# sj-shoff/ImageProcessor

Measured on AMD Instinct MI355X. Metric: images/sec (resize+thumb+watermark) on 1080p batch at 1/2/4/8 MI355X, higher is better.
Workload: dtype f32+f64

## Files before the change

### imageprocessor_amd/csrc/ipx_ks.h

```cpp
#pragma once

#include <vector>

#include "ipx_internal.h"

namespace ipx {

struct KsAxis {
    int dw = 0, sw = 0;
    int ntap = 0;
    std::vector<int32_t> lo, cnt;
    std::vector<double> w;
    std::vector<double> itw, itwffff;
    std::vector<double> ones;
};
bool ks_build_axis(int dw, int sw, KsAxis *out);

struct KsAxisDev {
    const int32_t *lo, *cnt;
    const double *w, *itw, *itwffff, *ones;
    int ntap;
};
size_t ks_axis_bytes(const KsAxis &a);
void ks_axis_pack(const KsAxis &a, uint8_t *h, const uint8_t *d, KsAxisDev *out);
// ... 18 lines not shown
    KsAxisDev ax, ay;
    int op;
    const int *opaque_flag;
    int kind;
    const uint8_t *src; int sstride; size_t src_fs;
    const uint8_t *cb, *cr; int cstride, ratio; size_t c_fs;
    int nframes;
};
hipError_t launch_ks_generic(const KsGenArgs &a, hipStream_t s);

}

namespace ipx {

struct KsStrip { int c0, c1, t0, tw; };
struct KsSeg { int ys, r0, r1; };
template <int NACC> struct KsRowT { double w[NACC], itw[NACC], ones[NACC]; int32_t emit[NACC]; float wf[NACC]; };
static_assert(sizeof(KsRowT<2>) == 64 && sizeof(KsRowT<4>) == 128, "row entries are copied dword-wise");

struct KsFusedOut {
    uint8_t *out; size_t frame_stride; int ostride, obytes;
    int dw, dh, sr_x0, sr_y0;
    int kind;
    int mode, aone;
    int pk;
    int ntap;
    int waves, cpl;
    int wcols;
    const double *wx;
    const float *wxf;
    int split, ntapf;
    float feps;
    const double *itwf;
    const int32_t *xlo;
    const int32_t *colb;
    const void *rows;
    const int32_t *rowoff;
};
struct KsFusedArgs {
    const uint8_t *src; size_t src_fs; int sstride, sw, sh;
    int src_kind;
    int taps_le_alpha;
    const uint8_t *cb, *cr; int cstride, ratio; size_t c_fs;
    uint8_t *wm; size_t wm_fs; int wm_stride;
    int nframes, nstrips, nseg, nthreads, pitch, dbuf;
    const KsStrip *strips; const KsSeg *segs;
    int nout; KsFusedOut o[2];
    int lds_w[2], lds_rows, lds_open;
    int open_per_wave;
    uint8_t wave_role[16];
    unsigned long long *stamps;
    int *redo;
    uint2 *fix; int *fix_count; int fix_cap[2], fix_stride;
};
struct KsFix { uint2 *list = nullptr; int *count = nullptr; int cap[2] = {0, 0}; KsAxisDev ax[2], ay[2]; };
struct KsFusedGeom { int nseg = 0; const KsSeg *segs = nullptr; const void *rows[2] = {nullptr, nullptr}; const int32_t *rowoff[2] = {nullptr, nullptr}; };
struct KsFusedPlan {
    bool ok = false;
    int nacc = 2, rows = 4, pitch = 0, nstrips = 0, nthreads = 0, nstg = 0, dbuf = 0;
    int lds_w[2] = {0, 0}, lds_rows = 0, lds_open = 0, lds_bytes = 0;
    struct Lds { int dbuf = 0, lds_w[2] = {0, 0}, lds_rows = 0, lds_open = 0, open_per_wave = 0, lds_bytes = 0; } fast;
    const KsStrip *strips = nullptr;
    struct Out { int ntap = 0, waves = 0, cpl = 0, wcols = 0; const double *wx = nullptr, *itwf = nullptr; const int32_t *xlo = nullptr, *colb = nullptr;
                 const float *wxf = nullptr; float feps = 0; int split = 1, ntapf = 0; } o[2];
    KsFusedGeom whole, split;
};
constexpr int kKsSplitRows = 96;
constexpr int kKsRows = 4;
constexpr int kKsMaxStage = 3;
constexpr int kKsMaxWaves = 12;
constexpr int kKsMaxThreads = 64 * kKsMaxWaves;
constexpr int kKsMaxCpl = 2;
constexpr int kKsSplitTaps = 16;
constexpr int kKsOpenPerWave = 128;
struct KsFusedIn { int dw, dh, sr_x0, sr_y0; const KsAxis *hx, *hy; int top_taps = 0; };
bool ks_fused_plan(int sw, int sh, const KsFusedIn *sc0, const KsFusedIn *sc1, int px_bytes, std::vector<uint8_t> *blob, KsFusedPlan *out);
void ks_fused_rebase(KsFusedPlan *p, const uint8_t *dev_blob);
hipError_t launch_ks_fused(const KsFusedPlan &p, KsFusedArgs &a, const KsFix *fix, int cus, hipStream_t s, bool *matched);
hipError_t launch_ks_fix(const KsGenArgs &g, const uint2 *list, size_t list_stride, const int *count, int count_stride, int cap, hipStream_t s);

}
```

### imageprocessor_amd/csrc/ipx_ks_fused.hip

```cpp
#include <algorithm>
#include <cstdio>
#include <cstdlib>
#include <type_traits>

#include "ipx_ks.h"

#pragma clang fp contract(off)

#include "ipx_device.h"

namespace ipx {
namespace {

#ifndef IPX_DIAG
#define IPX_DIAG 0
#endif
#if IPX_DIAG
#define KS_DIAG_ARGS , tsum, tlast
#define KS_STAMP(i) do { const unsigned long long t_ = __builtin_amdgcn_s_memtime(); tsum[i] += t_ - tlast; tlast = t_; } while (0)
#else
#define KS_DIAG_ARGS
#define KS_STAMP(i) do { } while (0)
#endif
constexpr int kOOB = 0x7fffffff;

__device__ __forceinline__ void ks_barrier() { asm volatile("s_waitcnt lgkmcnt(0)\n\ts_barrier" ::: "memory"); }
typedef uint32_t u32x4 __attribute__((ext_vector_type(4)));

__device__ __forceinline__ uint32_t ks_ftou8(double f)
{
    int i = (int)(0xffff * f + 0.5);
    i = min(max(i, 0), 0xffff);
    return (uint32_t)i >> 8;
}

enum { KS_RGBA = 0, KS_NRGBA = 1, KS_YCC = 2, KS_GRAY = 3, KS_TAP64 = 4 };
template <int SRC> struct KsPx { static constexpr int bytes = SRC == KS_RGBA ? 4 : SRC == KS_GRAY ? 2 : 8; };
enum { KS_TAP_PLAIN = 0,
       KS_TAP_CLAMP = 1,
       KS_TAP_TOP = 2,
       KS_TAP_MINTOP = 3 };

struct KsStageRegs { uint32_t v[4]; };

__device__ __forceinline__ void ks_ycc16(uint32_t yb, int rt, int gt, int bt, uint32_t &r, uint32_t &g, uint32_t &b)
{
    const int yy1 = (int)(yb * 0x10101u);
    r = (uint32_t)min(max((yy1 + rt) >> 8, 0), 0xffff);
    g = (uint32_t)min(max((yy1 + gt) >> 8, 0), 0xffff);
    b = (uint32_t)min(max((yy1 + bt) >> 8, 0), 0xffff);
}

template <int SRC>
// ... 391 lines not shown
                    }
                }
            }
        }
    }
}

template <int SRC, int NCH, int NACC, int B, bool OPQ, bool RAG, bool FAST>
__global__ __launch_bounds__(kKsMaxThreads) void ks_fused_kernel(KsFusedArgs a)
{
    typedef std::conditional_t<FAST, float, double> Sum;
    constexpr int CPLM = NACC == 2 ? kKsMaxCpl : 1;
    extern __shared__ __align__(16) uint8_t lds[];
    constexpr int PXB = KsPx<SRC>::bytes;
    constexpr int CHB = 4 * PXB;
    const int tid = (int)threadIdx.x, lane = tid & 63, wv = tid >> 6;
    int item = (int)blockIdx.x;
    if (!OPQ && !FAST && a.redo && !a.redo[item]) return;
    const int seg = item % a.nseg;
    item /= a.nseg;
    const int strip = item % a.nstrips, frame = item / a.nstrips;
    const KsStrip st = a.strips[strip];
    const KsSeg sg = a.segs[seg];
    const int pitch = a.pitch, CH = pitch / CHB;
    typedef KsRowT<NACC> Row;
    constexpr int RW = (int)(sizeof(Row) / 4);
    constexpr int SPX = SRC == KS_RGBA || SRC == KS_NRGBA ? 4 : SRC == KS_TAP64 ? 8 : 1;
    const int hs = SRC == KS_YCC && (a.ratio == IPX_YCBCR_422 || a.ratio == IPX_YCBCR_420), vs = SRC == KS_YCC && (a.ratio == IPX_YCBCR_420 || a.ratio == IPX_YCBCR_440);

    const uint8_t *sframe = a.src + (size_t)frame * a.src_fs;
    const __amdgpu_buffer_rsrc_t srs = __builtin_amdgcn_make_buffer_rsrc((void *)sframe, 0, (a.sh - 1) * a.sstride + a.sw * SPX, 0x00020000);
    const int chh = vs ? (a.sh + 1) / 2 : a.sh, cww = hs ? (a.sw + 1) / 2 : a.sw;
    const __amdgpu_buffer_rsrc_t cbrs = __builtin_amdgcn_make_buffer_rsrc((void *)(SRC == KS_YCC ? a.cb + (size_t)frame * a.c_fs : nullptr), 0,
                                                                         SRC == KS_YCC ? (chh - 1) * a.cstride + cww : 0, 0x00020000);
    const __amdgpu_buffer_rsrc_t crrs = __builtin_amdgcn_make_buffer_rsrc((void *)(SRC == KS_YCC ? a.cr + (size_t)frame * a.c_fs : nullptr), 0,
                                                                         SRC == KS_YCC ? (chh - 1) * a.cstride + cww : 0, 0x00020000);
    const __amdgpu_buffer_rsrc_t wrs = __builtin_amdgcn_make_buffer_rsrc((void *)(a.wm ? a.wm + (size_t)frame * a.wm_fs : nullptr), 0,
                                                                        a.wm ? (a.sh - 1) * a.wm_stride + a.sw * 4 : 0, 0x00020000);

    int s_lds[kKsMaxStage], s_src[kKsMaxStage], s_wm[kKsMaxStage], s_row[kKsMaxStage], s_cx[kKsMaxStage], s_np[kKsMaxStage];
    constexpr bool ragged = RAG && (SRC == KS_RGBA || SRC == KS_NRGBA);
#pragma unroll
    for (int i = 0; i < kKsMaxStage; i++) {
        const int q = tid + i * a.nthreads;
        const int row = q / CH, ch = q - row * CH, x = st.t0 + ch * 4;
        const bool in = q < B * CH && x < a.sw;
        s_row[i] = in ? row : -1;
        s_lds[i] = row * pitch + ch * CHB;
        s_src[i] = in ? row * a.sstride + x * SPX : kOOB;
        s_cx[i] = in ? (hs ? x >> 1 : x) : kOOB;
        s_np[i] = !ragged ? 4 : in ? min(4, a.sw - x) : 0;
        s_wm[i] = in && x >= st.c0 && x < st.c1 ? row * a.wm_stride + x * 4 : kOOB;
    }
    const int rk = tid / (B * RW), ri = tid - rk * (B * RW);
    const bool rstage = rk < a.nout;
    const uint32_t *rsrc = rstage ? (const uint32_t *)a.o[rk].rows + (size_t)a.o[rk].rowoff[seg] * RW + ri : nullptr;

    int role = -1, wk = 0;
    {
        const int rb = a.wave_role[wv & 15];
        if (rb != 0xff) { role = rb >> 4; wk = rb & 15; }
    }
    role = __builtin_amdgcn_readfirstlane(role);
    wk = __builtin_amdgcn_readfirstlane(wk);
    KsCol<NCH, NACC, Sum> col[CPLM];
    __amdgpu_buffer_rsrc_t ors = __builtin_amdgcn_make_buffer_rsrc((void *)nullptr, 0, 0, 0x00020000);
    int ntap = 0, wstride = 0, ostride = 0, cpl = 0, mode = KS_TAP_PLAIN;
    float feps = 0.f;
    bool split2 = false;
    bool aone = false;
    const uint8_t *rows_lds = lds + a.lds_rows;
    const int dbuf = a.dbuf;
    const int tile_bytes = B * pitch, rows_bytes = 2 * B * (int)sizeof(Row);
    if (role >= 0) {
        const KsFusedOut &o = a.o[role];
        ors = __builtin_amdgcn_make_buffer_rsrc((void *)(o.out + (size_t)frame * o.frame_stride), 0, o.obytes, 0x00020000);
        split2 = FAST && o.split == 2;
        ntap = FAST ? (split2 ? o.ntapf >> 1 : o.ntapf) : o.ntap;
        wstride = o.wcols * (FAST ? 4 : 8); ostride = o.ostride; cpl = o.cpl; feps = o.feps;
        mode = o.mode; aone = o.aone != 0;
        rows_lds += role * B * (int)sizeof(Row);
        const int cb = o.colb[strip], ce = o.colb[strip + 1];
        {
            const int n = (FAST ? o.ntapf : o.ntap) * o.wcols;
            if (FAST) {
                const float *wsrc = o.wxf + (size_t)strip * o.ntapf * o.wcols;
                float *wdst = (float *)(lds + a.lds_w[role]);
                for (int i = wk * 64 + lane; i < n; i += o.waves * 64) wdst[i] = wsrc[i];
            } else {
                const double *wsrc = o.wx + (size_t)strip * o.ntap * o.wcols;
                double *wdst = (double *)(lds + a.lds_w[role]);
                for (int i = wk * 64 + lane; i < n; i += o.waves * 64) wdst[i] = wsrc[i];
            }
        }
#pragma unroll
        for (int j = 0; j < CPLM; j++) {
            const int slot = wk * 64 + lane + j * 64 * o.waves;
            const int part = split2 ? slot & 1 : 0, cslot = split2 ? slot >> 1 : slot, dx = cb + cslot;
            const bool has = j < o.cpl && dx < ce;
            col[j].clear();
            col[j].itwf = has ? o.itwf[dx] : 0.0;
            col[j].xb = has ? (o.sr_x0 + o.xlo[dx] - st.t0 + part * ntap) * PXB : 0;
            col[j].wofs = a.lds_w[role] + (has ? cslot : 0) * (FAST ? 4 : 8) + part * ntap * wstride;
            col[j].ooff = has && part == 0 ? dx * 4 : kOOB;
        }
    }

    const int ngroups = (sg.r1 - sg.ys + B - 1) / B;
    KsStageRegs stage[kKsMaxStage];
    uint32_t stage2[SRC == KS_TAP64 ? kKsMaxStage : 1][4];
    uint32_t rstg = 0;
    auto issue = [&](int g) {
        const int y0 = sg.ys + g * B;
#pragma unroll
        for (int i = 0; i < kKsMaxStage; i++) {
            const bool ok = s_row[i] >= 0 && y0 + s_row[i] < sg.r1;
            const int off = ok ? s_src[i] : kOOB;
            if (SRC == KS_RGBA || SRC == KS_NRGBA || SRC == KS_TAP64) {
                u32x4 v = __builtin_amdgcn_raw_buffer_load_b128(srs, ragged && s_np[i] < 4 ? kOOB : off, y0 * a.sstride, 0);
                if (ragged) {
                    const int np = ok ? s_np[i] : 4;
                    v.x |= __builtin_amdgcn_raw_buffer_load_b32(srs, np < 4 ? off : kOOB, y0 * a.sstride, 0);
                    v.y |= __builtin_amdgcn_raw_buffer_load_b32(srs, np == 2 || np == 3 ? off + 4 : kOOB, y0 * a.sstride, 0);
                    v.z |= __builtin_amdgcn_raw_buffer_load_b32(srs, np == 3 ? off + 8 : kOOB, y0 * a.sstride, 0);
                }
                stage[i].v[0] = v.x; stage[i].v[1] = v.y; stage[i].v[2] = v.z; stage[i].v[3] = v.w;
                if (SRC == KS_TAP64) {
                    const u32x4 u = __builtin_amdgcn_raw_buffer_load_b128(srs, ok ? s_src[i] + 16 : kOOB, y0 * a.sstride, 0);
                    stage2[SRC == KS_TAP64 ? i : 0][0] = u.x; stage2[SRC == KS_TAP64 ? i : 0][1] = u.y;
                    stage2[SRC == KS_TAP64 ? i : 0][2] = u.z; stage2[SRC == KS_TAP64 ? i : 0][3] = u.w;
                }
            } else {
                stage[i].v[0] = __builtin_amdgcn_raw_buffer_load_b32(srs, off, y0 * a.sstride, 0);
                if (SRC == KS_YCC) {
                    const int cy = vs ? (y0 + s_row[i]) >> 1 : y0 + s_row[i];
                    const int coff = ok ? cy * a.cstride + s_cx[i] : kOOB;
                    if (hs) {
                        stage[i].v[1] = (uint32_t)(unsigned short)__builtin_amdgcn_raw_buffer_load_b16(cbrs, coff, 0, 0);
                        stage[i].v[2] = (uint32_t)(unsigned short)__builtin_amdgcn_raw_buffer_load_b16(crrs, coff, 0, 0);
                    } else {
                        stage[i].v[1] = __builtin_amdgcn_raw_buffer_load_b32(cbrs, coff, 0, 0);
                        stage[i].v[2] = __builtin_amdgcn_raw_buffer_load_b32(crrs, coff, 0, 0);
                    }
                }
            }
        }
        if (rstage) rstg = rsrc[(size_t)g * B * RW];
    };
    issue(0);
    bool bad = false;
    KsOpen open;
    if (FAST) {
        const int pk = role >= 0 ? a.o[role].pk : 0;
        open.wave = (uint2 *)(lds + a.lds_open) + wv * a.open_per_wave;
        open.n = 0; open.room = a.open_per_wave; open.full = false;
        open.list = a.fix + (size_t)frame * a.fix_stride + (pk ? a.fix_cap[0] : 0); open.count = a.fix_count + 2 * frame + pk; open.cap = a.fix_cap[pk];
    }
#if IPX_DIAG
    unsigned long long tsum[6] = {0, 0, 0, 0, 0, 0}, tlast = __builtin_amdgcn_s_memtime();
#endif
    for (int g = 0; g < ngroups; g++) {
#if IPX_DIAG
        asm volatile("s_waitcnt vmcnt(0)" ::: "memory");
        KS_STAMP(0);
#endif
        const int y0 = sg.ys + g * B, buf = dbuf ? g & 1 : 0;
#pragma unroll
        for (int i = 0; i < kKsMaxStage; i++) {
            if (s_row[i] < 0) continue;
            uint8_t *dst = lds + buf * tile_bytes + s_lds[i];
            u32x4 v;
            if (SRC == KS_TAP64) {
                const uint32_t *s0 = stage[i].v, *s1 = stage2[SRC == KS_TAP64 ? i : 0];
                *(u32x4 *)dst = u32x4{s0[0], s0[1], s0[2], s0[3]};
                *(u32x4 *)(dst + 16) = u32x4{s1[0], s1[1], s1[2], s1[3]};
                v.x = __builtin_amdgcn_perm(s0[1], s0[0], 0x07050301u); v.y = __builtin_amdgcn_perm(s0[3], s0[2], 0x07050301u);
                v.z = __builtin_amdgcn_perm(s1[1], s1[0], 0x07050301u); v.w = __builtin_amdgcn_perm(s1[3], s1[2], 0x07050301u);
            } else v = ks_convert<SRC>(stage[i], dst, hs);
            const int y = y0 + s_row[i];
            const bool live = y < sg.r1;
            if (OPQ && live) {
                uint32_t m = v.x & v.y & v.z & v.w;
                if (ragged && s_np[i] < 4) m = v.x & (s_np[i] > 1 ? v.y : ~0u) & (s_np[i] > 2 ? v.z : ~0u);
                bad |= (m >> 24) != 0xffu;
            }
            if (a.wm && live && y >= sg.r0) {
                if (!ragged) __builtin_amdgcn_raw_buffer_store_b128(v, wrs, s_wm[i], y0 * a.wm_stride, 0);
                else {
                    const int np = s_np[i], wo = s_wm[i];
                    __builtin_amdgcn_raw_buffer_store_b128(v, wrs, np == 4 ? wo : kOOB, y0 * a.wm_stride, 0);
                    __builtin_amdgcn_raw_buffer_store_b32(v.x, wrs, np < 4 ? wo : kOOB, y0 * a.wm_stride, 0);
                    __builtin_amdgcn_raw_buffer_store_b32(v.y, wrs, (np == 2 || np == 3) && wo != kOOB ? wo + 4 : kOOB, y0 * a.wm_stride, 0);
                    __builtin_amdgcn_raw_buffer_store_b32(v.z, wrs, np == 3 && wo != kOOB ? wo + 8 : kOOB, y0 * a.wm_stride, 0);
                }
            }
        }
        if (rstage) ((uint32_t *)(lds + a.lds_rows + buf * rows_bytes))[rk * B * RW + ri] = rstg;
        KS_STAMP(1);
        if (OPQ && g == 0) {
            if (__syncthreads_or(bad)) {
                if (tid == 0) a.redo[blockIdx.x] = 1;
                return;
            }
        } else ks_barrier();
        KS_STAMP(2);
        if (g + 1 < ngroups) issue(g + 1);
        KS_STAMP(3);
        if (role >= 0) {
            const uint8_t *tile = lds + buf * tile_bytes, *rws = rows_lds + buf * rows_bytes;
#define KS_COLS(MODE, AONE)                                                                                                              \
    _Pragma("unroll") for (int j = 0; j < CPLM; j++)                                                                                 \
        if (j < cpl) ks_column<SRC, NCH, NACC, B, MODE, AONE>(lds, tile, col[j], ntap, wstride, pitch, rws, ors, ostride KS_DIAG_ARGS)
#define KS_COLSF(MODE)                                                                                                                   \
    do {                                                                                                                                 \
        if (CPLM > 1 && cpl > 1) ks_columns_fast<SRC, NCH, NACC, B, MODE, CPLM>(lds, tile, col, ntap, wstride, pitch, rws, ors, ostride, feps, false, open KS_DIAG_ARGS); \
        else if (cpl > 0) ks_columns_fast<SRC, NCH, NACC, B, MODE, 1>(lds, tile, col, ntap, wstride, pitch, rws, ors, ostride, feps, split2, open KS_DIAG_ARGS);          \
    } while (0)
            if constexpr (FAST) {
                if constexpr (SRC == KS_YCC) {
                    if (!aone) { KS_COLSF(KS_TAP_TOP); }
                    else { KS_COLSF(KS_TAP_PLAIN); }
                } else if constexpr (SRC == KS_TAP64) {
                    if (mode == KS_TAP_MINTOP) { KS_COLSF(KS_TAP_TOP); }
                    else { KS_COLSF(KS_TAP_PLAIN); }
                } else if constexpr (SRC == KS_NRGBA) {
                    if (mode == KS_TAP_TOP) { KS_COLSF(KS_TAP_TOP); }
                    else { KS_COLSF(KS_TAP_PLAIN); }
                } else { KS_COLSF(KS_TAP_PLAIN); }
            } else if (SRC == KS_RGBA) {
                if (NCH == 4 && mode == KS_TAP_CLAMP) { KS_COLS(KS_TAP_CLAMP, false); }
                else { KS_COLS(KS_TAP_PLAIN, false); }
            } else if (SRC == KS_GRAY) {
                if (aone) { KS_COLS(KS_TAP_PLAIN, true); }
                else { KS_COLS(KS_TAP_PLAIN, false); }
            } else if (SRC == KS_YCC) {
                if (aone) { KS_COLS(KS_TAP_PLAIN, true); }
                else { KS_COLS(KS_TAP_TOP, false); }
// ... 201 lines not shown
```

### imageprocessor_amd/csrc/ipx_ks_host.cpp

```cpp
#include <algorithm>
#include <cmath>
#include <cstdlib>
#include <cstring>
#include <type_traits>

#include "ipx_ks.h"

namespace ipx {

bool ks_build_axis(int dw, int sw, KsAxis *out)
{
    if (dw <= 0 || sw <= 0) return false;
    const double support = 1.0;
    const double scale = (double)sw / (double)dw;
    double half_width = support, kernel_arg_scale = 1.0;
    if (scale > 1) {
        half_width *= scale;
        kernel_arg_scale = 1 / scale;
    }
    KsAxis &a = *out;
    a.dw = dw; a.sw = sw; a.ntap = 0;
    a.lo.assign(dw, 0); a.cnt.assign(dw, 0); a.itw.assign(dw, 0.0); a.itwffff.assign(dw, 0.0); a.ones.assign(dw, 0.0);
    std::vector<std::vector<double>> ws(dw);
    for (int x = 0; x < dw; x++) {
// ... 310 lines not shown
                for (int i = 0; i < colb[k][c + 1] - colb[k][c]; i++)
                    for (int t = 0; t < hx.ntap; t++)
                        wxf[((size_t)c * o.ntapf + t) * wcols[k] + i] = (float)(hx.w[(size_t)(colb[k][c] + i) * hx.ntap + t] * hx.itwffff[colb[k][c] + i] * unit);
            o.wxf = as_off<float>(blob_put(blob, wxf.data(), wxf.size() * sizeof(float)));
            o.feps = ks_float_eps(hx.ntap, sc[k]->hy->ntap);
            o.itwf = as_off<double>(blob_put(blob, hx.itwffff.data(), hx.itwffff.size() * sizeof(double)));
            o.xlo = as_off<int32_t>(blob_put(blob, hx.lo.data(), hx.lo.size() * sizeof(int32_t)));
            o.colb = as_off<int32_t>(blob_put(blob, colb[k].data(), colb[k].size() * sizeof(int32_t)));
        }
        for (int gi = 0; gi < 2; gi++) {
            KsFusedGeom &g = gi ? P.split : P.whole;
            std::vector<KsSeg> segs;
            make_segs(sh, gi ? std::max(1, (sh + split_rows / 2) / split_rows) : 1, sc, &segs);
            g.nseg = (int)segs.size();
            g.segs = as_off<KsSeg>(blob_put(blob, segs.data(), segs.size() * sizeof(KsSeg)));
            for (int k = 0; k < 2; k++) {
                if (!sc[k]) continue;
                std::vector<int32_t> rowoff;
                if (P.nacc == 2) {
                    std::vector<KsRowT<2>> rows;
                    build_rows<2>(*sc[k], segs, B, &rows, &rowoff);
                    g.rows[k] = as_off<void>(blob_put(blob, rows.data(), rows.size() * sizeof(rows[0])));
                } else {
                    std::vector<KsRowT<4>> rows;
                    build_rows<4>(*sc[k], segs, B, &rows, &rowoff);
                    g.rows[k] = as_off<void>(blob_put(blob, rows.data(), rows.size() * sizeof(rows[0])));
                }
                g.rowoff[k] = as_off<int32_t>(blob_put(blob, rowoff.data(), rowoff.size() * sizeof(int32_t)));
            }
        }
        P.ok = true;
        return true;
    }
    return false;
}

void ks_fused_rebase(KsFusedPlan *p, const uint8_t *d)
{
    auto fix = [&](auto *&ptr) { ptr = (std::remove_reference_t<decltype(ptr)>)(const void *)(d + (uintptr_t)ptr); };
    fix(p->strips);
    for (int k = 0; k < 2; k++) {
        if (!p->o[k].wx) continue;
        fix(p->o[k].wx); fix(p->o[k].itwf); fix(p->o[k].xlo); fix(p->o[k].colb); fix(p->o[k].wxf);
    }
    for (KsFusedGeom *g : {&p->whole, &p->split}) {
        fix(g->segs);
        for (int k = 0; k < 2; k++) {
            if (!g->rows[k] && !g->rowoff[k]) continue;
            fix(g->rows[k]); fix(g->rowoff[k]);
        }
    }
}

}
```

### imageprocessor_amd/csrc/ipx_runtime.hip

```cpp
#include <algorithm>
#include <chrono>
#include <condition_variable>
#include <cstdlib>
#include <cstring>
#include <map>
#include <mutex>
#include <new>
#include <thread>
#include <utility>
#include <vector>

#include "ipx_runtime_internal.h"
#include "ipx_ks.h"

#ifndef IPX_DIAG
#define IPX_DIAG 0
#endif

namespace {

struct ScalePrep {
    bool empty;
    Rect adr;
};
// ... 77 lines not shown
int dev_scale_src(ipx_ctx *ctx, hipStream_t s, int *flag, uint8_t *dst, int dw, int dh, int dstride, const Rect &dr,
                  const DevSrc &src, const Rect &sr, int op, size_t dst_fs = 0, int kind_override = -1, const KsAxisDev *axes = nullptr)
{
    ScalePrep pr;
    int rc = scale_prepare(dw, dh, dr, src.w, src.h, sr, op, &pr);
    if (rc) return rc;
    if (pr.empty) return IPX_OK;
    if (src.kind == IPX_SRC_YCBCR) op = IPX_OP_SRC;
    if (op == IPX_OP_OVER && src.kind == IPX_SRC_TAP64) IPX_HIP(launch_opaque_scan_tap64(src.pix, src.w, src.h, src.stride, flag, s));
    else if (op == IPX_OP_OVER) IPX_HIP(launch_opaque_scan(src.pix, src.w, src.h, src.stride, flag, s));
    KsGenArgs a{};
    if (axes) { a.ax = axes[0]; a.ay = axes[1]; }
    else {
        if ((rc = ks_axis_get(ctx, dr.dx(), sr.dx(), &a.ax))) return rc;
        if ((rc = ks_axis_get(ctx, dr.dy(), sr.dy(), &a.ay))) return rc;
    }
    a.dst = dst; a.dstride = dstride; a.src = src.pix; a.sstride = src.stride;
    a.dr_x0 = dr.x0; a.dr_y0 = dr.y0;
    a.adr_x0 = pr.adr.x0; a.adr_y0 = pr.adr.y0; a.adr_x1 = pr.adr.x1; a.adr_y1 = pr.adr.y1;
    a.sr_x0 = sr.x0; a.sr_y0 = sr.y0;
    a.op = op; a.opaque_flag = op == IPX_OP_OVER ? flag : nullptr;
    a.kind = kind_override >= 0 ? kind_override : src.kind;
    a.cb = src.cb; a.cr = src.cr; a.cstride = src.cstride; a.ratio = src.ratio;
    a.nframes = src.nframes; a.src_fs = src.frame_stride; a.c_fs = src.c_frame_stride; a.dst_fs = dst_fs;
    IPX_HIP(launch_ks_generic(a, s));
    return IPX_OK;
}

DevSrc rgba_src(const uint8_t *p, int w, int h, int stride, int kind = IPX_SRC_RGBA)
{
    DevSrc d;
    d.kind = kind; d.pix = p; d.stride = stride; d.w = w; d.h = h;
    return d;
}

int dev_draw(hipStream_t s, uint8_t *dst, int dw, int dh, int dstride, Rect r, const uint8_t *src,
             int sw, int sh, int sstride, int spx, int spy, int op)
{
    return dev_draw_src(s, dst, dw, dh, dstride, r, rgba_src(src, sw, sh, sstride), spx, spy, op);
}

int dev_scale(ipx_ctx *ctx, hipStream_t s, int *flag, uint8_t *dst, int dw, int dh, int dstride, const Rect &dr,
              const uint8_t *src, int sw, int sh, int sstride, const Rect &sr, int op)
{
    return dev_scale_src(ctx, s, flag, dst, dw, dh, dstride, dr, rgba_src(src, sw, sh, sstride), sr, op);
}

int glyphs_for_frame(const ipx_glyphset *gs, int dw, int dh, ClippedGlyphs *out)
{
    std::lock_guard<std::mutex> lk(gs->mu);
    auto it = gs->clipped.find({dw, dh});
    if (it != gs->clipped.end()) { *out = it->second; return IPX_OK; }
    std::vector<DevGlyph> tab;
    Rect bb{0, 0, 0, 0};
    for (const GlyphHost &g : gs->g) {
        Rect r = g.dr;
        int spx = 0, spy = 0, mpx = g.mpx, mpy = g.mpy;
        if (!draw_clip(r, dw, dh, false, 0, 0, spx, spy, true, g.mw, g.mh, mpx, mpy)) continue;
        DevGlyph d;
        d.mask = gs->masks_dev + g.mask_off + (size_t)mpy * g.mw + mpx;
        d.mstride = g.mw;
        d.x0 = r.x0; d.y0 = r.y0; d.x1 = r.x1; d.y1 = r.y1;
        if (tab.empty()) bb = r;
        else {
            bb.x0 = std::min(bb.x0, r.x0); bb.y0 = std::min(bb.y0, r.y0);
            bb.x1 = std::max(bb.x1, r.x1); bb.y1 = std::max(bb.y1, r.y1);
        }
        tab.push_back(d);
    }
    ClippedGlyphs c;
    c.n = (int)tab.size();
    c.bbox = bb;
    if (c.n) {
        IPX_HIP(hipMalloc((void **)&c.dev, tab.size() * sizeof(DevGlyph)));
        IPX_HIP(hipMemcpy(c.dev, tab.data(), tab.size() * sizeof(DevGlyph), hipMemcpyHostToDevice));
    }
    gs->clipped[{dw, dh}] = c;
    *out = c;
    return IPX_OK;
}

int dev_composite(hipStream_t s, uint8_t *dst, int dw, int dh, int dstride, size_t frame_stride,
                  int nframes, const ipx_glyphset *gs)
{
    ClippedGlyphs c;
    int rc = glyphs_for_frame(gs, dw, dh, &c);
    if (rc) return rc;
    IPX_HIP(launch_composite(dst, dstride, frame_stride, nframes, c.dev, c.n, c.bbox,
                             gs->col[0] * 0x101u, gs->col[1] * 0x101u, gs->col[2] * 0x101u,
                             gs->col[3] * 0x101u, s));
    return IPX_OK;
}

}

extern "C" {

static void prepare_hip_env();
int ipx_device_count(void) try
{
    prepare_hip_env();
    clear_error();
    int n = 0;
    hipError_t e = hipGetDeviceCount(&n);
    if (e != hipSuccess) { (void)hipGetLastError(); set_error("hipGetDeviceCount: %s", hipGetErrorString(e)); return IPX_ERR_NODEVICE; }
    return n;
}
IPX_CATCH_STATUS

static void prepare_hip_env()
{
    static std::once_flag once;
    std::call_once(once, [] {
        if (!getenv("GPU_MAX_HW_QUEUES")) {
            char v[16];
            snprintf(v, sizeof v, "%d", std::max(8, env_int("IPX_LANES", 5) + 3));
            setenv("GPU_MAX_HW_QUEUES", v, 0);
        }
    });
}

int ipx_create(const ipx_config *cfg, ipx_ctx **out) try
{
    clear_error();
    if (!out) { set_error("ipx_create: null out"); return IPX_ERR_INVALID; }
    *out = nullptr;
    prepare_hip_env();
    int ndev = 0;
// ... 344 lines not shown
{
    IPX_ENTER(ctx);
    IPX_FRAME("ipx_dev_scale_bilinear_rgba8", "destination", dst, dw, dh, dstride);
    IPX_FRAME("ipx_dev_scale_bilinear_rgba8", "source", src, sw, sh, sstride);
    hipStream_t s = stream ? (hipStream_t)stream : ctx->stream;
    int *flag = nullptr;
    if (op == IPX_OP_OVER) {
        IPX_HIP(hipMallocAsync((void **)&flag, sizeof(int), s));
    }
    int rc = dev_scale(ctx, s, flag, dst, dw, dh, dstride, to_rect(dr), src, sw, sh, sstride, to_rect(sr), op);
    if (flag) (void)hipFreeAsync(flag, s);
    return rc;
}
IPX_CATCH_STATUS

int ipx_dev_draw_rgba8(ipx_ctx *ctx, void *stream, uint8_t *dst, int dw, int dh, int dstride,
                       ipx_rect r, const uint8_t *src, int sw, int sh, int sstride, int spx, int spy,
                       int op) try
{
    IPX_ENTER(ctx);
    IPX_FRAME("ipx_dev_draw_rgba8", "destination", dst, dw, dh, dstride);
    IPX_FRAME("ipx_dev_draw_rgba8", "source", src, sw, sh, sstride);
    return dev_draw(stream ? (hipStream_t)stream : ctx->stream, dst, dw, dh, dstride, to_rect(r), src,
                    sw, sh, sstride, spx, spy, op);
}
IPX_CATCH_STATUS

int ipx_glyphset_create(ipx_ctx *ctx, const ipx_glyph *glyphs, int n, const uint8_t col[4],
                        ipx_glyphset **out) try
{
    IPX_ENTER(ctx);
    if (!out || n < 0 || (n && !glyphs) || !col) { set_error("ipx_glyphset_create: bad argument"); return IPX_ERR_INVALID; }
    if (n > kMaxGlyphs) { set_error("ipx_glyphset_create: %d glyphs exceed the limit of %d", n, kMaxGlyphs); return IPX_ERR_UNSUPPORTED; }
    *out = nullptr;
    ipx_glyphset *gs = new (std::nothrow) ipx_glyphset;
    if (!gs) { set_error("out of memory"); return IPX_ERR_NOMEM; }
    gs->device = ctx->device;
    memcpy(gs->col, col, 4);
    std::vector<uint8_t> blob;
    for (int i = 0; i < n; i++) {
        const ipx_glyph &g = glyphs[i];
        if (g.mw < 0 || g.mh < 0 || (g.mw && g.mh && (!g.mask || g.mstride < g.mw))) {
            set_error("ipx_glyphset_create: glyph %d has a bad mask", i);
            delete gs;
            return IPX_ERR_INVALID;
        }
        GlyphHost h;
        h.mask_off = blob.size();
        h.mw = g.mw; h.mh = g.mh; h.dr = to_rect(g.dr); h.mpx = g.mpx; h.mpy = g.mpy;
        for (int y = 0; y < g.mh; y++) blob.insert(blob.end(), g.mask + (size_t)y * g.mstride, g.mask + (size_t)y * g.mstride + g.mw);
        gs->g.push_back(h);
    }
    gs->masks_bytes = blob.size();
    if (!blob.empty()) {
        hipError_t e = hipMalloc((void **)&gs->masks_dev, blob.size());
        if (e == hipSuccess) e = hipMemcpy(gs->masks_dev, blob.data(), blob.size(), hipMemcpyHostToDevice);
        if (e != hipSuccess) {
            set_error("glyph mask upload failed: %s", hipGetErrorString(e));
            ipx_glyphset_destroy(ctx, gs);
            return IPX_ERR_HIP;
        }
    }
    *out = gs;
    return IPX_OK;
}
IPX_CATCH_STATUS

void ipx_glyphset_destroy(ipx_ctx *ctx, ipx_glyphset *gs)
{
    if (!gs) return;
    (void)hipSetDevice(ctx ? ctx->device : gs->device);
    for (auto &kv : gs->clipped) if (kv.second.dev) (void)hipFree(kv.second.dev);
    if (gs->masks_dev) (void)hipFree(gs->masks_dev);
    delete gs;
}

int ipx_dev_composite_glyphs_rgba8(ipx_ctx *ctx, void *stream, uint8_t *dst, int dw, int dh,
                                   int dstride, const ipx_glyphset *gs) try
{
    IPX_ENTER(ctx);
    if (!gs) { set_error("ipx_dev_composite_glyphs_rgba8: bad argument"); return IPX_ERR_INVALID; }
    IPX_FRAME("ipx_dev_composite_glyphs_rgba8", "destination", dst, dw, dh, dstride);
    return dev_composite(stream ? (hipStream_t)stream : ctx->stream, dst, dw, dh, dstride, 0, 1, gs);
}
IPX_CATCH_STATUS

int ipx_scale_bilinear_rgba8(ipx_ctx *ctx, uint8_t *dst, int dw, int dh, int dstride, ipx_rect dr,
                             const uint8_t *src, int sw, int sh, int sstride, ipx_rect sr, int op) try
{
    IPX_ENTER(ctx);
    IPX_FRAME("ipx_scale_bilinear_rgba8", "destination", dst, dw, dh, dstride);
    IPX_FRAME("ipx_scale_bilinear_rgba8", "source", src, sw, sh, sstride);
    ScalePrep pr;
    int rc = scale_prepare(dw, dh, to_rect(dr), sw, sh, to_rect(sr), op, &pr);
    if (rc) return rc;
    if (pr.empty || dw == 0 || dh == 0) return IPX_OK;
    LaneLease lane(ctx);
    const size_t sbytes = align256((size_t)sw * sh * 4), dbytes = align256((size_t)dw * dh * 4);
    rc = lane_reserve(lane.get(), sbytes + dbytes);
    if (rc) return rc;
    uint8_t *dsrc = lane->dev, *ddst = lane->dev + sbytes;
    hipStream_t s = lane->stream;
    if (sw && sh) IPX_HIP(hipMemcpy2DAsync(dsrc, (size_t)sw * 4, src, sstride, (size_t)sw * 4, sh, hipMemcpyHostToDevice, s));
    IPX_HIP(hipMemcpy2DAsync(ddst, (size_t)dw * 4, dst, dstride, (size_t)dw * 4, dh, hipMemcpyHostToDevice, s));
    rc = dev_scale(ctx, s, lane->flag, ddst, dw, dh, dw * 4, to_rect(dr), dsrc, sw, sh, sw * 4, to_rect(sr), op);
    if (rc) { (void)hipStreamSynchronize(s); return rc; }
    IPX_HIP(hipMemcpy2DAsync(dst, dstride, ddst, (size_t)dw * 4, (size_t)dw * 4, dh, hipMemcpyDeviceToHost, s));
    IPX_HIP(hipStreamSynchronize(s));
    return IPX_OK;
}
IPX_CATCH_STATUS

int ipx_draw_rgba8(ipx_ctx *ctx, uint8_t *dst, int dw, int dh, int dstride, ipx_rect r,
                   const uint8_t *src, int sw, int sh, int sstride, int spx, int spy, int op) try
{
    IPX_ENTER(ctx);
    IPX_FRAME("ipx_draw_rgba8", "destination", dst, dw, dh, dstride);
    IPX_FRAME("ipx_draw_rgba8", "source", src, sw, sh, sstride);
    if (op != IPX_OP_OVER && op != IPX_OP_SRC) { set_error("draw: unknown op %d", op); return IPX_ERR_INVALID; }
    if (!dw || !dh || !sw || !sh) return IPX_OK;
    LaneLease lane(ctx);
    const size_t sbytes = align256((size_t)sw * sh * 4), dbytes = align256((size_t)dw * dh * 4);
    int rc = lane_reserve(lane.get(), sbytes + dbytes);
    if (rc) return rc;
    uint8_t *dsrc = lane->dev, *ddst = lane->dev + sbytes;
// ... 402 lines not shown
    if (!plan) return;
    if (!cached) { ipx_plan_destroy(ctx, plan); return; }
    if (!ctx) return;
    std::lock_guard<std::mutex> lk(ctx->plan_mu);
    if (plan->cache_refs > 0) plan->cache_refs--;
}

int ipx_plan_query(const ipx_plan *plan, ipx_plan_info *info) try
{
    clear_error();
    if (!plan || !info) { set_error("ipx_plan_query: bad argument"); return IPX_ERR_INVALID; }
    *info = plan->info;
    return IPX_OK;
}
IPX_CATCH_STATUS

static int plan_src_status(const char *who, const ipx_plan *pl, long long stride, int bpp)
{
    if (frame_span_ok(pl->p.sw, pl->p.sh, stride, bpp)) return IPX_OK;
    set_error("%s: %dx%d frames with a row stride of %lld bytes are beyond the 2 GiB span the kernels address", who, pl->p.sw, pl->p.sh, stride);
    return IPX_ERR_UNSUPPORTED;
}
#define IPX_PLAN_SRC(who, pl, stride, bpp) do { const int rc_ = plan_src_status(who, pl, stride, bpp); if (rc_) return rc_; } while (0)

static hipError_t composite_text(const ipx_plan *pl, uint8_t *wm, size_t wm_frame_stride, int n, hipStream_t s)
{
    if (!wm || pl->glyphs.n <= 0 || !pl->p.glyphs) return hipSuccess;
    const uint8_t *c = pl->p.glyphs->col;
    return launch_composite(wm, pl->p.sw * 4, wm_frame_stride, n, pl->glyphs.dev, pl->glyphs.n, pl->glyphs.bbox, c[0] * 0x101u, c[1] * 0x101u,
                            c[2] * 0x101u, c[3] * 0x101u, s);
}

static int run_dev_any(ipx_ctx *ctx, hipStream_t s, const ipx_plan *pl, int n, const DevSrc &src, uint8_t *resize_out, size_t resize_frame_stride,
                       uint8_t *thumb_out, size_t thumb_frame_stride, uint8_t *wm_out, size_t wm_frame_stride)
{
    const int sw = pl->p.sw, sh = pl->p.sh;
    uint8_t *outs[2] = {pl->sc[0].on ? resize_out : nullptr, pl->sc[1].on ? thumb_out : nullptr};
    const size_t ostr[2] = {resize_frame_stride, thumb_frame_stride};
    uint8_t *wm = pl->p.do_watermark ? wm_out : nullptr;
    for (int k = 0; k < 2; k++)
        if (pl->sc[k].dw <= 0 || pl->sc[k].dh <= 0) outs[k] = nullptr;
    if (!wm && !outs[0] && !outs[1]) return IPX_OK;
    int kinds[2] = {src.kind, pl->p.crop_to_fit ? ks_crop_kind(src.kind) : src.kind};

    const bool gray = src.kind == IPX_SRC_YCBCR && src.cstride == 0;
    const KsFusedPlan &fp = pl->fused[src.kind == IPX_SRC_RGBA ? 0 : gray ? 2 : 1];
    if (fp.ok && env_int("IPX_FUSED", 1)) {
        KsFusedArgs a{};
        a.src = src.pix; a.src_fs = src.frame_stride; a.sstride = src.stride; a.sw = sw; a.sh = sh;
        a.src_kind = src.kind; a.cb = src.cb; a.cr = src.cr; a.cstride = src.cstride; a.ratio = src.ratio; a.c_fs = src.c_frame_stride;
        a.wm = wm; a.wm_fs = wm_frame_stride; a.wm_stride = sw * 4;
        a.nframes = n;
        a.taps_le_alpha = src.le_alpha;
        for (int k = 0; k < 2; k++) {
            if (!outs[k]) continue;
            const PlanScale &ps = pl->sc[k];
            KsFusedOut &o = a.o[a.nout++];
            o.out = outs[k]; o.frame_stride = ostr[k]; o.ostride = ps.dw * 4; o.obytes = ps.dw * ps.dh * 4;
            o.dw = ps.dw; o.dh = ps.dh; o.sr_x0 = ps.sr.x0; o.sr_y0 = ps.sr.y0;
            o.kind = kinds[k]; o.pk = k;
        }
        int *redo = nullptr;
        KsFix fixv, *fix = nullptr;
        const int max_items = n * fp.nstrips * std::max(fp.whole.nseg, fp.split.nseg);
        const bool spec = src.kind == IPX_SRC_RGBA && env_int("IPX_KS_SPEC", 1);
        const bool fast = (spec || src.kind == IPX_SRC_YCBCR || src.kind == IPX_SRC_NRGBA || (src.kind == IPX_SRC_TAP64 && src.le_alpha)) &&
                          env_int("IPX_KS_FAST", 1) != 0;
        if (spec || fast) {
            const int cap_env = env_int("IPX_KS_FIX_CAP", 0);
            int cap[2] = {0, 0};
            for (int k = 0; k < 2; k++)
                if (fast && outs[k]) cap[k] = cap_env > 0 ? cap_env : (int)std::min<size_t>(std::max<size_t>((size_t)pl->sc[k].dw * pl->sc[k].dh / 96, 256), (size_t)1 << 20);
            const size_t flags = align256((size_t)max_items * sizeof(int)), counts = fast ? align256((size_t)n * 2 * sizeof(int)) : 0;
            IPX_HIP(hipMallocAsync((void **)&redo, flags + counts + (size_t)n * (cap[0] + cap[1]) * sizeof(uint2), s));
            if (fast) {
                fixv.count = (int *)((uint8_t *)redo + flags);
                fixv.list = (uint2 *)((uint8_t *)redo + flags + counts);
                fixv.cap[0] = cap[0]; fixv.cap[1] = cap[1];
                for (int k = 0; k < 2; k++) { fixv.ax[k] = pl->sc[k].ax[0]; fixv.ay[k] = pl->sc[k].ax[1]; }
                IPX_HIP(hipMemsetAsync(fixv.count, 0, (size_t)n * 2 * sizeof(int), s));
                fix = &fixv;
            }
        }
        a.redo = redo;
#if IPX_DIAG
        static unsigned long long *stamp_buf = nullptr;
        if (env_int("IPX_STAMPS", 0)) {
            if (!stamp_buf) IPX_HIP(hipMalloc((void **)&stamp_buf, 24 * sizeof(unsigned long long)));
            IPX_HIP(hipMemsetAsync(stamp_buf, 0, 24 * sizeof(unsigned long long), s));
            a.stamps = stamp_buf;
        }
#endif
        bool matched = false;
        hipError_t e = launch_ks_fused(fp, a, fix, ctx->cus, s, &matched);
        if (fix && matched && e == hipSuccess && env_int("IPX_KS_STATS", 0)) {
            std::vector<int> cnt((size_t)n * 2), flags((size_t)max_items);
            (void)hipMemcpyAsync(cnt.data(), fixv.count, cnt.size() * sizeof(int), hipMemcpyDeviceToHost, s);
            (void)hipMemcpyAsync(flags.data(), redo, flags.size() * sizeof(int), hipMemcpyDeviceToHost, s);
            (void)hipStreamSynchronize(s);
            long long tot[2] = {0, 0}; int mx[2] = {0, 0}, nredo = 0;
            for (int i = 0; i < n; i++) for (int k = 0; k < 2; k++) { tot[k] += cnt[2 * i + k]; mx[k] = std::max(mx[k], cnt[2 * i + k]); }
            for (int f : flags) nredo += f != 0;
            fprintf(stderr, "[ipx ks stats] %d frames: undecided pixels per frame resize mean %.1f max %d (room %d), thumbnail mean %.1f max %d (room %d); %d of %d items redone in float64\n", n,
                    (double)tot[0] / n, mx[0], fixv.cap[0], (double)tot[1] / n, mx[1], fixv.cap[1], nredo, max_items);
        }
        if (redo) (void)hipFreeAsync(redo, s);
#if IPX_DIAG
        if (a.stamps && matched) {
            unsigned long long h[24];
            IPX_HIP(hipMemcpyAsync(h, a.stamps, sizeof h, hipMemcpyDeviceToHost, s));
            IPX_HIP(hipStreamSynchronize(s));
            const char *who[3] = {"resize waves", "thumbnail waves", "idle waves"};
            for (int r = 0; r < 3; r++) {
                double tot = 0;
                for (int i = 0; i < 6; i++) tot += (double)h[r * 8 + i];
                if (tot > 0)
                    fprintf(stderr, "[ipx stamps] %-16s share of wave time: wait-loads %.1f%%  drain %.1f%%  barrier %.1f%%  issue %.1f%%  scaleX %.1f%%  scaleY %.1f%%  (%.3g cycles)\n", who[r],
                            100 * h[r * 8] / tot, 100 * h[r * 8 + 1] / tot, 100 * h[r * 8 + 2] / tot, 100 * h[r * 8 + 3] / tot, 100 * h[r * 8 + 4] / tot, 100 * h[r * 8 + 5] / tot, tot);
            }
        }
#endif
        if (e != hipSuccess) { set_error("one-pass kernel launch failed: %s", hipGetErrorString(e)); return IPX_ERR_HIP; }
        if (matched) {
            IPX_HIP(composite_text(pl, wm, wm_frame_stride, n, s));
            return IPX_OK;
        }
    }

    if (wm) {
        const int rc = dev_draw_src(s, wm, sw, sh, sw * 4, Rect{0, 0, sw, sh}, src, 0, 0, IPX_OP_SRC, wm_frame_stride);
        if (rc) return rc;
        IPX_HIP(composite_text(pl, wm, wm_frame_stride, n, s));
    }
    for (int k = 0; k < 2; k++) {
        if (!outs[k]) continue;
        const PlanScale &ps = pl->sc[k];
        const int rc = dev_scale_src(ctx, s, nullptr, outs[k], ps.dw, ps.dh, ps.dw * 4, Rect{0, 0, ps.dw, ps.dh}, src, ps.sr, IPX_OP_SRC, ostr[k],
                                     kinds[k], ps.ax);
        if (rc) return rc;
    }
    return IPX_OK;
}

int ipx_plan_run_dev(ipx_ctx *ctx, void *stream, const ipx_plan *pl, int n, const uint8_t *src,
                     int sstride, size_t src_frame_stride, uint8_t *resize_out,
                     size_t resize_frame_stride, uint8_t *thumb_out, size_t thumb_frame_stride,
                     uint8_t *wm_out, size_t wm_frame_stride) try
{
    IPX_ENTER(ctx);
    if (!pl || n < 0 || !src || (long long)sstride < (long long)pl->p.sw * 4) {
        set_error("ipx_plan_run_dev: bad argument");
        return IPX_ERR_INVALID;
    }
    IPX_PLAN_SRC("ipx_plan_run_dev", pl, sstride, 4);
    if (n == 0) return IPX_OK;
    if (n > 65535) { set_error("ipx_plan_run_dev: at most 65535 frames per call"); return IPX_ERR_UNSUPPORTED; }
    DevSrc d = rgba_src(src, pl->p.sw, pl->p.sh, sstride);
    d.nframes = n; d.frame_stride = src_frame_stride;
    return run_dev_any(ctx, stream ? (hipStream_t)stream : ctx->stream, pl, n, d, resize_out, resize_frame_stride, thumb_out, thumb_frame_stride,
                       wm_out, wm_frame_stride);
}
IPX_CATCH_STATUS

constexpr int kPalettedKind = 100;
constexpr int kDeepKind = 200;
static int deep_bpp(int kind) { return kind == IPX_DEEP_GRAY16 ? 2 : (kind == IPX_DEEP_CMYK ? 4 : 8); }
static int run_host_packed(ipx_ctx *ctx, const ipx_plan *pl, int n, int kind, const uint8_t *src, int sstride, size_t src_frame_stride,
                           const uint8_t *palettes, uint8_t *resize_out, size_t resize_frame_stride, uint8_t *thumb_out,
                           size_t thumb_frame_stride, uint8_t *wm_out, size_t wm_frame_stride, const char *who)
{
    const int sw = pl->p.sw, sh = pl->p.sh;
    const int bpp = kind >= kDeepKind ? deep_bpp(kind - kDeepKind) : (kind == IPX_SRC_RGBA || kind == IPX_SRC_NRGBA ? 4 : 1);
    auto dstride = [](size_t bytes) { return (bytes & 15) == 0 ? bytes : align256(bytes); };
    const size_t fsrc = dstride((size_t)sw * sh * bpp);
    const size_t fpal = kind == kPalettedKind ? 1024 : 0;
    const size_t fres = resize_out ? dstride(pl->info.resize_bytes) : 0;
    const size_t fth = thumb_out ? dstride(pl->info.thumb_bytes) : 0;
// ... 406 lines not shown
```

### imageprocessor_amd/csrc/ipx_runtime_internal.h

```cpp
#pragma once

#include <sched.h>

#include <algorithm>
#include <cctype>
#include <cstdio>
#include <condition_variable>
#include <cstdlib>
#include <cstring>
#include <deque>
#include <map>
#include <mutex>
#include <string>
#include <utility>
#include <vector>

#include "ipx_internal.h"
#include "ipx_ks.h"

using namespace ipx;

struct Lane {
    hipStream_t stream = nullptr;
    uint8_t *dev = nullptr;
    size_t dev_bytes = 0;
    int *flag = nullptr;
    uint8_t *dec = nullptr;
    size_t dec_bytes = 0;
    uint8_t *pin = nullptr;
    size_t pin_bytes = 0;
    hipEvent_t ev[3] = {nullptr, nullptr, nullptr};
    bool busy = false;
};

struct ipx_ctx {
    int device = 0;
    int cus = 256;
    hipStream_t stream = nullptr;
    std::vector<Lane> lanes;
    size_t lane_bytes = 0;
    std::mutex mu;
    std::condition_variable cv;
    std::mutex host_mu;
    std::map<void *, size_t> host_size;
    std::multimap<size_t, void *> host_free_blocks;
    std::deque<void *> host_lru;
    size_t host_cached = 0, host_cache_limit = (size_t)8 << 30;
    int jj_active = 0;
    uint8_t *flat_chroma = nullptr;
    std::mutex plan_mu;
    std::map<std::string, std::pair<ipx_glyphset *, ipx_plan *>> plan_cache;
    uint64_t plan_clock = 0;
    std::mutex ks_mu;
    std::map<std::pair<int, int>, std::pair<uint8_t *, KsAxisDev>> ks_axes;
    static constexpr size_t kFlatChromaBytes = (size_t)64 << 10;
};

struct GlyphHost {
    size_t mask_off;
    int mw, mh;
    Rect dr;
    int mpx, mpy;
};

struct ClippedGlyphs {
    DevGlyph *dev = nullptr;
    int n = 0;
    Rect bbox{0, 0, 0, 0};
};

struct ipx_glyphset {
    int device = 0;
    std::vector<GlyphHost> g;
    uint8_t *masks_dev = nullptr;
    size_t masks_bytes = 0;
    uint8_t col[4] = {0, 0, 0, 0};
    mutable std::mutex mu;
    mutable std::map<std::pair<int, int>, ClippedGlyphs> clipped;
};

struct PlanScale {
    bool on = false;
    int dw = 0, dh = 0;
    Rect sr{0, 0, 0, 0};
    KsAxis hx, hy;
    KsAxisDev ax[2]{};
};

struct ipx_plan {
    ipx_plan_params p{};
    ipx_plan_info info{};
    PlanScale sc[2];
    KsFusedPlan fused[3];
    uint8_t *blob = nullptr;
    ClippedGlyphs glyphs;
    mutable std::mutex mu;
    ipx_glyphset *owned_gs = nullptr;
    int cache_refs = 0;
    uint64_t cache_stamp = 0;
};

inline int env_int(const char *name, int dflt)
{
    const char *v = getenv(name);
    return v && *v ? atoi(v) : dflt;
}

struct DeviceGuard {
    explicit DeviceGuard(int dev) { ok = hipSetDevice(dev) == hipSuccess; }
    bool ok;
};

#define IPX_ENTER(ctx)                                                         \
    clear_error();                                                             \
    if (!(ctx)) { set_error("%s: null context", __func__); return IPX_ERR_INVALID; } \
    DeviceGuard guard_((ctx)->device);                                         \
    if (!guard_.ok) { set_error("hipSetDevice(%d) failed", (ctx)->device); return IPX_ERR_HIP; }

class LaneLease {
public:
    explicit LaneLease(ipx_ctx *c) : c_(c)
    {
        std::unique_lock<std::mutex> lk(c->mu);
        c->cv.wait(lk, [&] {
            for (auto &l : c->lanes) if (!l.busy) return true;
            return false;
        });
        for (auto &l : c->lanes) if (!l.busy) { l.busy = true; lane_ = &l; break; }
// ... 136 lines not shown
```

Measured before the change: 255,400.

## Fuse glyph text compositing into the one-pass resize/watermark kernel

```diff
diff --git a/imageprocessor_amd/csrc/ipx_ks.h b/imageprocessor_amd/csrc/ipx_ks.h
--- a/imageprocessor_amd/csrc/ipx_ks.h
+++ b/imageprocessor_amd/csrc/ipx_ks.h
@@ -94,7 +94,11 @@
     unsigned long long *stamps;
     int *redo;
     uint2 *fix; int *fix_count; int fix_cap[2], fix_stride;
+    const DevGlyph *gl; int ngl; Rect gbox; uint32_t gcol[4];
+    const uint8_t *gmask; int gmask_bytes;
 };
+constexpr int kKsTextHits = 2;
+int ks_text_hits(const Rect *g, int n);
 struct KsFix { uint2 *list = nullptr; int *count = nullptr; int cap[2] = {0, 0}; KsAxisDev ax[2], ay[2]; };
 struct KsFusedGeom { int nseg = 0; const KsSeg *segs = nullptr; const void *rows[2] = {nullptr, nullptr}; const int32_t *rowoff[2] = {nullptr, nullptr}; };
 struct KsFusedPlan {
diff --git a/imageprocessor_amd/csrc/ipx_ks_fused.hip b/imageprocessor_amd/csrc/ipx_ks_fused.hip
--- a/imageprocessor_amd/csrc/ipx_ks_fused.hip
+++ b/imageprocessor_amd/csrc/ipx_ks_fused.hip
@@ -1,4 +1,5 @@
 #include <algorithm>
+#include <cstddef>
 #include <cstdio>
 #include <cstdlib>
 #include <type_traits>
@@ -496,6 +497,23 @@
         s_np[i] = !ragged ? 4 : in ? min(4, a.sw - x) : 0;
         s_wm[i] = in && x >= st.c0 && x < st.c1 ? row * a.wm_stride + x * 4 : kOOB;
     }
+    const bool text = a.ngl > 0 && a.wm && st.c0 < a.gbox.x1 && st.c1 > a.gbox.x0 && sg.r0 < a.gbox.y1 && sg.r1 > a.gbox.y0;
+    typedef const __attribute__((address_space(4))) int KsConstInt;
+    KsConstInt *gtab = (KsConstInt *)(const void *)a.gl;
+    constexpr int GLW = (int)(sizeof(DevGlyph) / 4);
+    static_assert(kKsTextHits == 2 && offsetof(DevGlyph, mask) == 0, "a chunk's glyphs go to slot 0, then slot 1");
+    uint32_t tm[kKsMaxStage][kKsTextHits];
+    int gtx = 0, gty = 0, gtm = 0, gts = 0;
+    if (text && lane < a.ngl) {
+        KsConstInt *gp = gtab + lane * GLW;
+        const int gx0 = gp[offsetof(DevGlyph, x0) / 4];
+        const uint64_t mk = (uint64_t)(uint32_t)gp[0] | (uint64_t)(uint32_t)gp[1] << 32;
+        gtx = gx0 | gp[offsetof(DevGlyph, x1) / 4] << 16;
+        gty = gp[offsetof(DevGlyph, y0) / 4] | gp[offsetof(DevGlyph, y1) / 4] << 16;
+        gts = gp[offsetof(DevGlyph, mstride) / 4];
+        gtm = (int)(mk - (uint64_t)(uintptr_t)a.gmask) - (gx0 & ~3);
+    }
+    bool tgrp = false;
     const int rk = tid / (B * RW), ri = tid - rk * (B * RW);
     const bool rstage = rk < a.nout;
     const uint32_t *rsrc = rstage ? (const uint32_t *)a.o[rk].rows + (size_t)a.o[rk].rowoff[seg] * RW + ri : nullptr;
@@ -554,7 +572,7 @@
     KsStageRegs stage[kKsMaxStage];
     uint32_t stage2[SRC == KS_TAP64 ? kKsMaxStage : 1][4];
     uint32_t rstg = 0;
-    auto issue = [&](int g) {
+    auto issue = [&](int g) __attribute__((always_inline)) {
         const int y0 = sg.ys + g * B;
 #pragma unroll
         for (int i = 0; i < kKsMaxStage; i++) {
@@ -590,6 +608,45 @@
             }
         }
         if (rstage) rstg = rsrc[(size_t)g * B * RW];
+        tgrp = text && y0 < a.gbox.y1 && y0 + B > a.gbox.y0;
+        int tx[kKsMaxStage];
+        bool inbox = false;
+#pragma unroll
+        for (int i = 0; i < kKsMaxStage; i++) {
+            const int q = tid + i * a.nthreads, row = q / CH;
+            tx[i] = tgrp && s_wm[i] != kOOB ? st.t0 + (q - row * CH) * 4 : kOOB;
+            inbox |= tx[i] != kOOB && tx[i] < a.gbox.x1 && tx[i] + 4 > a.gbox.x0;
+        }
+        tgrp = __builtin_amdgcn_readfirstlane((int)(__ballot(inbox) != 0)) != 0;
+        if (tgrp) {
+            int nh[kKsMaxStage], off[kKsMaxStage][kKsTextHits];
+#pragma unroll
+            for (int i = 0; i < kKsMaxStage; i++) {
+                nh[i] = 0;
+#pragma unroll
+                for (int h = 0; h < kKsTextHits; h++) off[i][h] = kOOB;
+            }
+            for (int k = 0; k < a.ngl; k++) {
+                const int ky = __builtin_amdgcn_readlane(gty, k), gy0 = ky & 0xffff, gy1 = ky >> 16;
+                if (gy1 <= y0 || gy0 >= y0 + B) continue;
+                const int kx = __builtin_amdgcn_readlane(gtx, k), gx0 = kx & 0xffff, gx1 = kx >> 16;
+                const int ms = __builtin_amdgcn_readlane(gts, k), mbase = __builtin_amdgcn_readlane(gtm, k);
+#pragma unroll
+                for (int i = 0; i < kKsMaxStage; i++) {
+                    const int y = y0 + s_row[i], x = tx[i];
+                    const bool hit = s_row[i] >= 0 && x != kOOB && y >= gy0 && y < gy1 && y >= sg.r0 && y < sg.r1 && x < gx1 && x + 4 > gx0;
+                    const int o = mbase + (y - gy0) * ms + x;
+                    off[i][0] = hit && nh[i] == 0 ? o : off[i][0];
+                    off[i][kKsTextHits - 1] = hit && nh[i] > 0 ? o : off[i][kKsTextHits - 1];
+                    nh[i] += hit;
+                }
+            }
+            const __amdgpu_buffer_rsrc_t mrs = __builtin_amdgcn_make_buffer_rsrc((void *)a.gmask, 0, a.gmask_bytes, 0x00020000);
+#pragma unroll
+            for (int i = 0; i < kKsMaxStage; i++)
+#pragma unroll
+                for (int h = 0; h < kKsTextHits; h++) tm[i][h] = __builtin_amdgcn_raw_buffer_load_b32(mrs, off[i][h], 0, 0);
+        }
     };
     issue(0);
     bool bad = false;
@@ -627,6 +684,17 @@
                 uint32_t m = v.x & v.y & v.z & v.w;
                 if (ragged && s_np[i] < 4) m = v.x & (s_np[i] > 1 ? v.y : ~0u) & (s_np[i] > 2 ? v.z : ~0u);
                 bad |= (m >> 24) != 0xffu;
+            }
+            if (tgrp) {
+                uint32_t px[4] = {v.x, v.y, v.z, v.w};
+#pragma unroll
+                for (int h = 0; h < kKsTextHits; h++)
+#pragma unroll
+                    for (int j = 0; j < 4; j++) {
+                        const uint32_t m = (tm[i][h] >> (8 * j)) & 0xffu;
+                        if (m) px[j] = glyph_over(px[j], m, a.gcol[0], a.gcol[1], a.gcol[2], a.gcol[3]);
+                    }
+                v = u32x4{px[0], px[1], px[2], px[3]};
             }
             if (a.wm && live && y >= sg.r0) {
                 if (!ragged) __builtin_amdgcn_raw_buffer_store_b128(v, wrs, s_wm[i], y0 * a.wm_stride, 0);
diff --git a/imageprocessor_amd/csrc/ipx_ks_host.cpp b/imageprocessor_amd/csrc/ipx_ks_host.cpp
--- a/imageprocessor_amd/csrc/ipx_ks_host.cpp
+++ b/imageprocessor_amd/csrc/ipx_ks_host.cpp
@@ -386,4 +386,25 @@
     }
 }
 
-}
+int ks_text_hits(const Rect *g, int n)
+{
+    if (n <= 0) return 0;
+    Rect bb = g[0];
+    for (int i = 1; i < n; i++) {
+        bb.x0 = std::min(bb.x0, g[i].x0); bb.y0 = std::min(bb.y0, g[i].y0);
+        bb.x1 = std::max(bb.x1, g[i].x1); bb.y1 = std::max(bb.y1, g[i].y1);
+    }
+    int most = 0;
+    std::vector<std::pair<int, int>> ev;
+    for (int cx = bb.x0 & ~3; cx < bb.x1; cx += 4) {
+        ev.clear();
+        for (int i = 0; i < n; i++)
+            if (cx < g[i].x1 && cx + 4 > g[i].x0 && g[i].y0 < g[i].y1) { ev.push_back({g[i].y0, 1}); ev.push_back({g[i].y1, -1}); }
+        std::sort(ev.begin(), ev.end());
+        int k = 0;
+        for (const auto &e : ev) most = std::max(most, k += e.second);
+    }
+    return most;
+}
+
+}
diff --git a/imageprocessor_amd/csrc/ipx_runtime.hip b/imageprocessor_amd/csrc/ipx_runtime.hip
--- a/imageprocessor_amd/csrc/ipx_runtime.hip
+++ b/imageprocessor_amd/csrc/ipx_runtime.hip
@@ -153,6 +153,9 @@
     auto it = gs->clipped.find({dw, dh});
     if (it != gs->clipped.end()) { *out = it->second; return IPX_OK; }
     std::vector<DevGlyph> tab;
+    std::vector<Rect> rects;
+    std::vector<const uint8_t *> srcs;
+    std::vector<int> mws;
     Rect bb{0, 0, 0, 0};
     for (const GlyphHost &g : gs->g) {
         Rect r = g.dr;
@@ -168,13 +171,37 @@
             bb.x1 = std::max(bb.x1, r.x1); bb.y1 = std::max(bb.y1, r.y1);
         }
         tab.push_back(d);
+        rects.push_back(r);
+        srcs.push_back(gs->masks_host.data() + g.mask_off + (size_t)mpy * g.mw + mpx);
+        mws.push_back(g.mw);
     }
     ClippedGlyphs c;
     c.n = (int)tab.size();
     c.bbox = bb;
+    c.hits = ks_text_hits(rects.data(), c.n);
     if (c.n) {
         IPX_HIP(hipMalloc((void **)&c.dev, tab.size() * sizeof(DevGlyph)));
         IPX_HIP(hipMemcpy(c.dev, tab.data(), tab.size() * sizeof(DevGlyph), hipMemcpyHostToDevice));
+        std::vector<uint8_t> km;
+        std::vector<size_t> koff;
+        for (int i = 0; i < c.n; i++) {
+            const Rect &r = rects[i];
+            const int xa = r.x0 & ~3, st = (r.x1 - xa + 3) & ~3;
+            koff.push_back(km.size());
+            km.resize(km.size() + (size_t)st * r.dy(), 0);
+            for (int y = 0; y < r.dy(); y++)
+                memcpy(km.data() + koff[i] + (size_t)y * st + (r.x0 - xa), srcs[i] + (size_t)y * mws[i], (size_t)r.dx());
+            tab[i].mstride = st;
+        }
+        if (!km.empty()) {
+            if (km.size() > 0x7fffffffu) return IPX_ERR_UNSUPPORTED;
+            c.kmask_bytes = (int)km.size();
+            IPX_HIP(hipMalloc((void **)&c.kmasks, km.size()));
+            IPX_HIP(hipMemcpy(c.kmasks, km.data(), km.size(), hipMemcpyHostToDevice));
+        }
+        for (int i = 0; i < c.n; i++) tab[i].mask = c.kmasks + koff[i];
+        IPX_HIP(hipMalloc((void **)&c.kdev, tab.size() * sizeof(DevGlyph)));
+        IPX_HIP(hipMemcpy(c.kdev, tab.data(), tab.size() * sizeof(DevGlyph), hipMemcpyHostToDevice));
     }
     gs->clipped[{dw, dh}] = c;
     *out = c;
@@ -625,6 +652,7 @@
         gs->g.push_back(h);
     }
     gs->masks_bytes = blob.size();
+    gs->masks_host = blob;
     if (!blob.empty()) {
         hipError_t e = hipMalloc((void **)&gs->masks_dev, blob.size());
         if (e == hipSuccess) e = hipMemcpy(gs->masks_dev, blob.data(), blob.size(), hipMemcpyHostToDevice);
@@ -643,7 +671,11 @@
 {
     if (!gs) return;
     (void)hipSetDevice(ctx ? ctx->device : gs->device);
-    for (auto &kv : gs->clipped) if (kv.second.dev) (void)hipFree(kv.second.dev);
+    for (auto &kv : gs->clipped) {
+        if (kv.second.dev) (void)hipFree(kv.second.dev);
+        if (kv.second.kdev) (void)hipFree(kv.second.kdev);
+        if (kv.second.kmasks) (void)hipFree(kv.second.kmasks);
+    }
     if (gs->masks_dev) (void)hipFree(gs->masks_dev);
     delete gs;
 }
@@ -1152,6 +1184,13 @@
         a.wm = wm; a.wm_fs = wm_frame_stride; a.wm_stride = sw * 4;
         a.nframes = n;
         a.taps_le_alpha = src.le_alpha;
+        const bool tail = env_int("IPX_KS_TAIL", 0) != 0;
+        if (wm && pl->glyphs.n > 0 && pl->glyphs.kdev && pl->glyphs.kmasks && pl->p.glyphs && pl->glyphs.hits <= kKsTextHits && pl->glyphs.n <= 64 && sw < 65536 && sh < 65536 && !tail) {
+            const uint8_t *c = pl->p.glyphs->col;
+            a.gl = pl->glyphs.kdev; a.ngl = pl->glyphs.n; a.gbox = pl->glyphs.bbox;
+            a.gmask = pl->glyphs.kmasks; a.gmask_bytes = pl->glyphs.kmask_bytes;
+            for (int k = 0; k < 4; k++) a.gcol[k] = c[k] * 0x101u;
+        }
         for (int k = 0; k < 2; k++) {
             if (!outs[k]) continue;
             const PlanScale &ps = pl->sc[k];
@@ -1222,7 +1261,7 @@
 #endif
         if (e != hipSuccess) { set_error("one-pass kernel launch failed: %s", hipGetErrorString(e)); return IPX_ERR_HIP; }
         if (matched) {
-            IPX_HIP(composite_text(pl, wm, wm_frame_stride, n, s));
+            if (a.ngl == 0) IPX_HIP(composite_text(pl, wm, wm_frame_stride, n, s));
             return IPX_OK;
         }
     }
diff --git a/imageprocessor_amd/csrc/ipx_runtime_internal.h b/imageprocessor_amd/csrc/ipx_runtime_internal.h
--- a/imageprocessor_amd/csrc/ipx_runtime_internal.h
+++ b/imageprocessor_amd/csrc/ipx_runtime_internal.h
@@ -67,6 +67,10 @@
     DevGlyph *dev = nullptr;
     int n = 0;
     Rect bbox{0, 0, 0, 0};
+    int hits = 0;
+    DevGlyph *kdev = nullptr;
+    uint8_t *kmasks = nullptr;
+    int kmask_bytes = 0;
 };
 
 struct ipx_glyphset {
@@ -74,6 +78,7 @@
     std::vector<GlyphHost> g;
     uint8_t *masks_dev = nullptr;
     size_t masks_bytes = 0;
+    std::vector<uint8_t> masks_host;
     uint8_t col[4] = {0, 0, 0, 0};
     mutable std::mutex mu;
     mutable std::map<std::pair<int, int>, ClippedGlyphs> clipped;
```

Measured after the change: 249,100 (median of 6 runs). 2.5% lower.
